# BGU-CS-VIL/DPMMSubClusters.jl

Hardware: AMD Instinct MI355X
Metric: Gibbs iterations/sec, N=10M D=64 NIW (higher is better)
Workload: dtype f32

## Files before the change

### dpmmsubclusters.jl_amd/binding.py

```python
import ctypes
import os
import subprocess

import numpy as np

_HERE = os.path.dirname(os.path.abspath(__file__))
PRIOR_NIW, PRIOR_MULT = 0, 1
MAX_CLUSTERS = 1024

_c_i64p = ctypes.POINTER(ctypes.c_int64)
_c_f32p = ctypes.POINTER(ctypes.c_float)
_c_f64p = ctypes.POINTER(ctypes.c_double)

ABI = [
    ("dpmm_abi_version", ctypes.c_int, []),
    ("dpmm_create", ctypes.c_int, [ctypes.POINTER(ctypes.c_void_p), ctypes.c_int, ctypes.c_int, ctypes.c_int64, ctypes.c_int64, ctypes.c_int, ctypes.c_uint64]),
    ("dpmm_destroy", ctypes.c_int, [ctypes.c_void_p]),
    ("dpmm_last_error", ctypes.c_char_p, [ctypes.c_void_p]),
    ("dpmm_upload_points", ctypes.c_int, [ctypes.c_void_p, _c_f32p, ctypes.c_int64]),
    ("dpmm_upload_points_device", ctypes.c_int, [ctypes.c_void_p, ctypes.c_void_p, ctypes.c_int64]),
    ("dpmm_upload_points_npy", ctypes.c_int, [ctypes.c_void_p, ctypes.c_void_p, ctypes.c_int, ctypes.c_int64, ctypes.c_int]),
    ("dpmm_upload_points_csc", ctypes.c_int, [ctypes.c_void_p, _c_i64p, _c_i64p, _c_f32p, ctypes.c_int]),
    ("dpmm_init_labels", ctypes.c_int, [ctypes.c_void_p, ctypes.c_int, ctypes.c_uint32]),
    ("dpmm_set_labels", ctypes.c_int, [ctypes.c_void_p, _c_i64p, _c_i64p]),
# ... 72 lines not shown
    ("dpmm_comm_allgather_host", ctypes.c_int, [ctypes.c_void_p, ctypes.c_void_p, ctypes.c_int64, ctypes.c_void_p]),
]

ABI_TENSOR = [
    ("dpmm_upload_points_strided_device", ctypes.c_int, [ctypes.c_void_p, ctypes.c_void_p, ctypes.c_int, ctypes.c_int64, ctypes.c_int64, ctypes.c_int]),
    ("dpmm_get_points_device", ctypes.c_int, [ctypes.c_void_p, ctypes.c_void_p, ctypes.c_int64]),
    ("dpmm_get_labels_device", ctypes.c_int, [ctypes.c_void_p, ctypes.c_void_p, ctypes.c_void_p]),
    ("dpmm_set_labels_device", ctypes.c_int, [ctypes.c_void_p, ctypes.c_void_p, ctypes.c_void_p]),
    ("dpmm_predict_points_device", ctypes.c_int, [ctypes.c_void_p, ctypes.c_void_p, ctypes.c_void_p]),
]
DT_F16, DT_BF16, DT_F32, DT_F64, DT_U8, DT_I16, DT_I32, DT_I64 = range(8)

HOST_ALLREDUCE_FN = ctypes.CFUNCTYPE(ctypes.c_int, ctypes.c_void_p, ctypes.c_void_p, ctypes.c_int64, ctypes.c_int)

MASTER_NSCALARS = 8
OPT_SCREEN_MARGIN, OPT_TAIL_SCREEN, OPT_PRESCREEN, OPT_ORDERED_SWEEP, OPT_MULT_FORCE_F32, OPT_STATS_ITEMS, OPT_STATS_GROUPS, OPT_TRACE_SLOW, OPT_LOGLIK_REF_CONST, OPT_WAVE_PRIO, OPT_MULT_NO_U8, OPT_SWEEP_GRID, OPT_SWEEP_QUEUE_ROUNDS, OPT_BALL_SCREEN, OPT_KERNEL_TIMING, OPT_STATS_DERIVE, OPT_NOISE_AHEAD, OPT_REF_BRACKET, OPT_SORT_TILE, OPT_ONE_COLLECTIVE, OPT_BF16_SCREENS, OPT_COMM_TIMEOUT_MS, OPT_DIRECTION_SCREEN, _OPT_RESERVED_24, OPT_MULT_DRAWS_AHEAD, OPT_B3_SUBLABELS, OPT_LEAN_TILES, OPT_MASTER_POLL, OPT_CHAIN_FUSION, OPT_LEAN_DIRECTION, OPT_PAIR_BALL = range(1, 32)


class DpmmError(RuntimeError):
    def __init__(self, code, msg):
        super().__init__(f"libdpmmhip error {code}: {msg}")
        self.code = code


def lib_path():
    return os.path.join(_HERE, "lib", "libdpmmhip.so")


def locked_make(args, lock_dir):
    import fcntl
    os.makedirs(lock_dir, exist_ok=True)
# ... 541 lines not shown
```

### dpmmsubclusters.jl_amd/csrc/dpmm_api.cpp

```cpp
#include "../../include/dpmm_hip.h"
#include "../../include/dpmm_hip_master.h"
#include "../../include/dpmm_hip_debug.h"
#include "../../include/dpmm_hip_tensor.h"

#include <hip/hip_runtime.h>
#include <dlfcn.h>

#include <algorithm>
#include <atomic>
#include <condition_variable>
#include <mutex>
#include <thread>
#include <chrono>
#include <cmath>
#include <cstdio>
#include <cstring>
#include <cstdlib>
#include <ctime>
#include <string>
#include <unordered_map>
#include <vector>

#include "dpmm_kernels.h"

// ... 114 lines not shown
    int sel_all_ones = 0, sel_capacity = 0;
    long long *d_counts64 = nullptr;
    float *d_malpha = nullptr;
    bool mult_master = false, mult_has_alpha1 = false;
    int rows_full_K = -1;
    double mult_prior_c[4] = {0, 0, 0, 0};
    int32_t *d_mpairs = nullptr;
    std::vector<int32_t> mpairs_req, mpairs_shadow;
    bool marg_req = false, marg_valid = false;
    int marg_req_outlier = 0, marg_K = 0, marg_np = 0;
    double *h_marg = nullptr;
    double *d_ccache = nullptr;
    bool cache_force = true;
    int cache_K = -1;
    int opt_derive = 1;
    int64_t dbg_early_wait = 0;
    int opt_noise_ahead = -1;
    bool master = false;
    NiwMasterArgs ma{};
    double *d_m0 = nullptr, *d_psi_lo = nullptr, *d_pairs = nullptr;
    double *d_Y[2] = {nullptr, nullptr};
    float *d_mu_draw[2] = {nullptr, nullptr};
    int draw_cur = 0;
    size_t pair_cap = 0;
    float *d_ld_sigma[2] = {nullptr, nullptr};
    int master_slots = 0, master_K = 0;
    hipStream_t stream2 = nullptr;
    hipEvent_t ev_master = nullptr, ev_spec = nullptr;
    hipEvent_t ev_noise = nullptr;
    hipEvent_t ev_pairs = nullptr;
// ... 145 lines not shown
    return e;
}

static int ensure_pinned(dpmm_ctx *c, size_t bytes) {
    if (bytes <= c->h_pin_bytes) return DPMM_OK;
    HIPCHK(c, sync_stream(c, c->stream));
    if (c->h_pin) hipHostFree(c->h_pin);
    c->h_pin = nullptr; c->h_pin_bytes = 0;
    size_t cap = 1 << 20;
    while (cap < bytes) cap *= 2;
    HIPCHK(c, hipHostMalloc((void **)&c->h_pin, cap, hipHostMallocDefault));
    c->h_pin_bytes = cap;
    return DPMM_OK;
}

static int fail(dpmm_ctx *c, int code, const std::string &msg) {
    if (c) c->err = msg; else g_create_error = msg;
    return code;
}

struct UidByValue { char internal[128]; };
namespace {
struct Rccl {
    void *handle = nullptr;
    int (*GetUniqueId)(void *) = nullptr;
    int (*CommInitRank)(void **, int,  UidByValue, int) = nullptr;
    int (*CommDestroy)(void *) = nullptr;
    int (*CommAbort)(void *) = nullptr;
    int (*AllReduce)(const void *, void *, size_t, int, int, void *, hipStream_t) = nullptr;
    int (*AllGather)(const void *, void *, size_t, int, void *, hipStream_t) = nullptr;
// ... 507 lines not shown
        if (int rc2 = pack_sparse_image(c, c->d_raw, c->d_Rp, c->K)) return rc2;
        c->rp_current = false;
        c->mspec_valid = false;
        HIPCHK(c, sync_stream(c, c->stream));
    }
    c->have_points = true;
    c->cache_force = true;
    c->rows_full_K = -1;
    return DPMM_OK;
}

int dpmm_init_labels(dpmm_ctx *c, int init_clusters, uint32_t epoch) {
    if (!c) return DPMM_EINVAL;
    if (init_clusters < 1 || init_clusters > DPMM_MAX_CLUSTERS) return fail(c, DPMM_ELIMIT, "init_clusters out of range");
    HIPCHK(c, hipSetDevice(c->device));
    if (c->n > 0) HIPCHK(c, launch_init_labels(c->dbins, c->n, c->first, init_clusters, 0, c->seed, epoch, c->stream));
    c->have_labels = true;
    c->rows_full_K = -1;
    return DPMM_OK;
}

int dpmm_init_labels_from(dpmm_ctx *c, int init_clusters, int first_label, uint32_t epoch) {
    if (!c) return DPMM_EINVAL;
    if (first_label < 1 || init_clusters < 1 || first_label - 1 + init_clusters > DPMM_MAX_CLUSTERS) return fail(c, DPMM_ELIMIT, "init_clusters / first_label out of range");
    HIPCHK(c, hipSetDevice(c->device));
    if (c->n > 0) HIPCHK(c, launch_init_labels(c->dbins, c->n, c->first, init_clusters, first_label - 1, c->seed, epoch, c->stream));
    c->have_labels = true;
    c->rows_full_K = -1;
    return DPMM_OK;
}

int dpmm_set_labels(dpmm_ctx *c, const int64_t *labels, const int64_t *sub) {
    if (!c) return DPMM_EINVAL;
    if (!c->have_labels && (!labels || !sub)) return fail(c, DPMM_ESTATE, "first dpmm_set_labels must provide both vectors");
    HIPCHK(c, hipSetDevice(c->device));
    if (c->n == 0) { c->have_labels = true; return DPMM_OK; }
    int64_t *tmp = nullptr;
    HIPCHK(c, hipMalloc(&tmp, sizeof(int64_t) * 2 * (size_t)c->n));
    int rc = DPMM_OK;
    hipError_t e = hipSuccess;
    if (labels) e = hipMemcpyAsync(tmp, labels, sizeof(int64_t) * c->n, hipMemcpyHostToDevice, c->stream);
    if (e == hipSuccess && sub) e = hipMemcpyAsync(tmp + c->n, sub, sizeof(int64_t) * c->n, hipMemcpyHostToDevice, c->stream);
    if (e == hipSuccess) e = launch_bins_from_i64(c->dbins, labels ? tmp : nullptr, sub ? tmp + c->n : nullptr, c->n, c->stream);
    if (e == hipSuccess) e = sync_stream(c, c->stream);
    hipFree(tmp);
    if (e != hipSuccess) { c->err = std::string("dpmm_set_labels: ") + hipGetErrorString(e); rc = DPMM_EHIP; }
    else c->have_labels = true;
    c->rows_full_K = -1;
    return rc;
}

int dpmm_get_labels(dpmm_ctx *c, int64_t *labels, int64_t *sub) {
    if (!c) return DPMM_EINVAL;
    if (!c->have_labels) return fail(c, DPMM_ESTATE, "labels not initialised");
    HIPCHK(c, hipSetDevice(c->device));
    if (c->n == 0) return DPMM_OK;
    int64_t *tmp = nullptr;
// ... 279 lines not shown
    for (char *p = bus; *p; ++p) if (*p >= 'A' && *p <= 'F') *p = (char)(*p - 'A' + 'a');
    const std::string path = std::string("/sys/bus/pci/devices/") + bus + "/numa_node";
    FILE *f = fopen(path.c_str(), "r");
    if (!f) return -1;
    int node = -1;
    if (fscanf(f, "%d", &node) != 1) node = -1;
    fclose(f);
    return node;
}

static int noise_flush(dpmm_ctx *c);
static int run_sweep(dpmm_ctx *c, uint32_t epoch, int final_argmax, float *table, int64_t table_stride) {
    if (!c->have_points || !c->have_params) return fail(c, DPMM_ESTATE, "sweep needs points and parameters");
    HIPCHK(c, hipSetDevice(c->device));
    if (c->n == 0) return DPMM_OK;
    if (c->prior == DPMM_PRIOR_NIW && !table) {
        if (!c->work_zeroed) HIPCHK(c, hipMemsetAsync(c->d_work, 0, sizeof(unsigned long long) * DPMM_WORK_SLOTS, c->stream));
        c->work_zeroed = false;
    }
    if (!table && (c->opt_timing & 1)) HIPCHK(c, hipEventRecord(c->ev[0], c->stream));
    if (c->prior == DPMM_PRIOR_NIW) {
        NiwSweepArgs a{};
        a.X = c->dX; a.ldx = c->ldx; a.n = c->n; a.first_index = c->first; a.ntiles = c->ntiles; a.K = c->K;
        a.Rp = c->d_Rp; a.mup = c->d_mup; a.cst = c->d_cst;
        a.tdf = c->predictive ? c->d_tdf : nullptr;
        a.scratch = table ? table : c->d_scratch;
        a.scratch_stride = table ? table_stride : c->scratch_stride;
        a.scratch_by_tile = table ? 1 : 0;
        a.labels_only = table ? 1 : 0;
        a.bins = c->dbins; a.seed = c->seed; a.epoch = epoch; a.final_argmax = final_argmax;
// ... 47 lines not shown
            if (parts && !c->ev_part[0]) for (auto &e : c->ev_part) HIPCHK(c, hipEventCreate(&e));
            if (use_lean) {
                const size_t hw = hard_list_words(c->n);
                uint32_t *mine = c->d_hard + (size_t)c->hard_flip * hw, *other = c->d_hard + (size_t)(c->hard_flip ^ 1) * hw;
                c->hard_flip ^= 1;
                c->lean_ran = true;
                uint32_t *need2 = a.need ? c->h_need + 8 * (size_t)c->sweep_grid_max : nullptr;
                const bool al = a.order != nullptr && c->perm_nbins > 0 && c->perm_nbins <= NIW_LEAN_MAX_BINS;
                uint32_t *need3 = a.need ? c->h_need + 12 * (size_t)c->sweep_grid_max : nullptr;
                NiwSweepArgs al_args = a;
                if (!c->opt_lean_dir) { al_args.sp_frag = nullptr; al_args.sp_cons = nullptr; }
                if (c->have_pb && c->opt_pair_ball && al_args.ball) al_args.ball |= 2;
                HIPCHK(c, launch_niw_lean(al_args, mine, need2, other, al ? c->sb.bin_start : nullptr, al ? c->perm_nbins : 0, need3, c->sweep_grid, c->stream));
                if (parts) HIPCHK(c, hipEventRecord(c->ev_part[0], c->stream));
                list = mine;
            }
            a.bf16scr |= 4;
            a.tdf = reinterpret_cast<const float *>(list);
            const float *mdist_kept = a.mdist;
            if (list) a.mdist = reinterpret_cast<const float *>(c->h_hard);
            HIPCHK(c, launch_niw_sweep(c->NB, a, c->sweep_grid, c->stream));
            a.mdist = mdist_kept;
            if (parts) HIPCHK(c, hipEventRecord(c->ev_part[1], c->stream));
            c->have_parts = parts ? (use_lean ? 2 : 1) : 0;
            a.bf16scr &= 3;
            a.tdf = nullptr;
            if (!list) HIPCHK(c, launch_niw_sub(a, nullptr, nullptr, c->sweep_grid, c->stream));
        } else {
            HIPCHK(c, launch_niw_sweep(c->NB, a, c->sweep_grid, c->stream));
            if (!table) c->have_parts = 0;
// ... 140 lines not shown
    HIPCHK(c, sync_stream(c, c->stream));
    c->rows_late = false;
    if (c->h_out) hipHostFree(c->h_out);
    c->h_out = nullptr; c->h_out_bytes = 0;
    size_t cap = 1 << 20;
    while (cap < bytes) cap *= 2;
    HIPCHK(c, hipHostMalloc((void **)&c->h_out, cap, hipHostMallocDefault));
    c->h_out_bytes = cap;
    return DPMM_OK;
}

static int flush_undo(dpmm_ctx *c) {
    if (!c->undo_pending) return DPMM_OK;
    c->undo_pending = false;
    const uint8_t *flags = reinterpret_cast<const uint8_t *>(c->d_out) + sizeof(double) * 2 * (size_t)c->K * (size_t)c->packed_stride;
    HIPCHK(c, launch_niw_undo_reset(c->dbins, c->n, c->K, flags, c->d_cside, c->stream));
    return DPMM_OK;
}
static int run_stats(dpmm_ctx *c, const int64_t *idx, int n_idx, bool with_reset = false, uint32_t reset_epoch = 0, uint8_t *flags_to = nullptr,
                     bool *flags_sent = nullptr) {
    if (!c->have_points || !c->have_labels || c->K < 1) return fail(c, DPMM_ESTATE, "suffstats need points, labels and parameters (K)");
    HIPCHK(c, hipSetDevice(c->device));
    const int nbins = 2 * c->K;
    c->marg_valid = false;
    c->mspec_valid = false;
    const bool one_auto = c->packed_stride <= 4096;
    const bool one_coll = with_reset && comm_attached(c) && (c->opt_one_collective < 0 ? one_auto : c->opt_one_collective != 0);
    c->last_pass_one_collective = one_coll;
    if (c->opt_timing & 2) HIPCHK(c, hipEventRecord(c->ev[2], c->stream));
    if (idx) {
// ... 10 lines not shown
        c->sel_all_ones = 0;
    } else if (with_reset && c->n > 0 && c->opt_derive) {
    } else if (c->sel_all_ones < nbins) {
        HIPCHK(c, hipMemsetAsync(c->sb.bin_sel, 1, c->sel_capacity, c->stream));
        c->sel_all_ones = c->sel_capacity;
    }
    bool derive = false;
    StatsArgs a{};
    a.X = c->dX; a.ldx = c->ldx; a.n = c->n; a.D = c->D; a.nbins = nbins; a.chunk = c->chunk;
    a.max_items = (int)((c->n + c->chunk - 1) / c->chunk) + nbins;
    a.range_groups = c->opt_stats_groups;
    a.sb = c->sb; a.slabs = c->d_slabs; a.slab_stride = c->slab_stride; a.out = (one_coll && c->prior == DPMM_PRIOR_NIW) ? c->d_red : c->d_out; a.packed_stride = c->packed_stride; a.row_off = c->d_row_off; a.inv_off = c->d_inv_off;
    if (with_reset && c->n > 0) {
        const bool fold_reset = (c->opt_chain & 8) != 0 && (c->n >= 4000000 || (c->opt_chain & 32) != 0) && nbins <= STEP_SPEC_MAX_BINS &&
                                c->sb.tile_spec != nullptr && c->sb.spec_bins != nullptr;
        HIPCHK(c, launch_step_hist(c->dbins, c->n, nbins, c->sb, c->stream, fold_reset ? 1 : 0, c->first, c->seed, reset_epoch));
        const long long *gc = nullptr;
        if (comm_attached(c) && !one_coll) {
            HIPCHK(c, launch_widen_counts(c->sb.fast_total, FAST_TOTAL_STRIDE, c->d_counts64, nbins, c->stream));
            if (int rc = comm_allreduce(c, c->d_counts64, nbins, 0)) return rc;
            gc = c->d_counts64;
        }
        uint8_t *flags = reinterpret_cast<uint8_t *>(c->d_out) + sizeof(double) * (size_t)nbins * (size_t)c->packed_stride;
        if (!fold_reset) HIPCHK(c, launch_step_reset(c->dbins, c->n, c->first, nbins, c->sb, gc, flags, c->K, c->seed, reset_epoch, one_coll ? c->d_cside : nullptr, c->stream));
        derive = c->opt_derive != 0;
        const int force_all = (c->cache_force || c->cache_K != c->K) ? 1 : 0;
        const StepReset rs{gc, flags, c->K, one_coll ? c->d_cside : nullptr, c->first, c->seed, reset_epoch};
        HIPCHK(c, launch_step_scan_scatter(c->dbins, a, derive ? 1 : 0, force_all, c->opt_chain & 1, fold_reset ? &rs : nullptr, c->stream));
        if (derive) { c->sel_all_ones = 0; c->cache_force = false; c->cache_K = c->K; }
    } else {
        if (c->n > 0) {
// ... 313 lines not shown
static bool master_marks_left(const double *sm, int K) { return master_records_marked(sm, 3 * (int64_t)K); }
static void master_mark_records(double *sm, int64_t nrec) {
    for (int64_t r = 0; r < nrec; ++r)
        for (int e = 0; e < 5; ++e) std::memcpy(&sm[r * DPMM_MASTER_NSCALARS + e], &MASTER_MARK, 8);
}
static int wait_master_records(dpmm_ctx *c, const double *sm, int64_t nrec, const double *pr, int64_t npr) {
    const bool armed = c->watchdog && c->coll_pending;
    if (armed) wd_arm(c);
    int rc = DPMM_OK;
    const auto t0 = std::chrono::steady_clock::now();
    auto next_query = t0 + std::chrono::milliseconds(1);
    std::chrono::steady_clock::time_point drained{};
    bool is_drained = false;
    for (uint64_t spin = 0;; ++spin) {
        if (!master_records_marked(sm, nrec) && !(npr > 0 && master_records_marked(pr, npr))) break;
        __builtin_ia32_pause();
        if ((spin & 63u) != 63u) continue;
        if (c->comm_aborted.load(std::memory_order_relaxed)) break;
        const auto now = std::chrono::steady_clock::now();
        if (now < next_query) continue;
        next_query = now + std::chrono::milliseconds(1);
        const hipError_t q = hipStreamQuery(c->stream);
        if (q == hipSuccess) {
            if (!is_drained) { is_drained = true; drained = now; ++c->dbg_early_wait; }
            else if (now - drained > std::chrono::seconds(5)) { rc = fail(c, DPMM_EHIP, "posterior records missing 5 s after the stream drained"); break; }
        } else if (q != hipErrorNotReady) { c->err = std::string("hipStreamQuery while waiting for the posteriors: ") + hipGetErrorString(q); rc = DPMM_EHIP; break; }
    }
    if (armed && wd_disarm(c)) {
        c->err = "collective timed out: a peer rank is gone or stuck (communicator aborted after DPMM_OPT_COMM_TIMEOUT_MS)";
        return DPMM_ECOMM;
    }
// ... 578 lines not shown
    }
    if (int rc = ensure_pinned(c, sizeof(int32_t) * h.size())) return rc;
    HIPCHK(c, sync_stream(c, c->stream));
    memcpy(c->h_pin, h.data(), sizeof(int32_t) * h.size());
    HIPCHK(c, launch_copy_bytes(c->d_small, c->h_pin, sizeof(int32_t) * h.size(), c->stream));
    return DPMM_OK;
}

int dpmm_split(dpmm_ctx *c, const int64_t *idx, const int64_t *new_idx, int n, uint32_t epoch) {
    if (!c) return DPMM_EINVAL;
    if (!c->have_labels) return fail(c, DPMM_ESTATE, "labels not initialised");
    if (n == 0) return DPMM_OK;
    if (!idx || !new_idx) return fail(c, DPMM_EINVAL, "null index list");
    HIPCHK(c, hipSetDevice(c->device));
    if (int rc = upload_idx(c, idx, new_idx, n, DPMM_MAX_CLUSTERS)) return rc;
    if (c->n > 0) HIPCHK(c, launch_split(c->dbins, c->n, c->first, c->d_small, n, c->seed, epoch, c->stream));
    c->rows_full_K = -1;
    return DPMM_OK;
}

int dpmm_merge(dpmm_ctx *c, const int64_t *idx, const int64_t *new_idx, int n) {
    if (!c) return DPMM_EINVAL;
    if (!c->have_labels) return fail(c, DPMM_ESTATE, "labels not initialised");
    if (n == 0) return DPMM_OK;
    if (!idx || !new_idx) return fail(c, DPMM_EINVAL, "null index list");
    HIPCHK(c, hipSetDevice(c->device));
    if (int rc = upload_idx(c, idx, new_idx, n, DPMM_MAX_CLUSTERS)) return rc;
    if (c->n > 0) HIPCHK(c, launch_merge(c->dbins, c->n, c->d_small, n, c->stream));
    c->rows_full_K = -1;
    return DPMM_OK;
}

int dpmm_remove_empty(dpmm_ctx *c, const int64_t *pts_count, int K) {
    if (!c) return DPMM_EINVAL;
    if (!c->have_labels) return fail(c, DPMM_ESTATE, "labels not initialised");
    if (!pts_count || K < 1 || K > DPMM_MAX_CLUSTERS) return fail(c, DPMM_EINVAL, "bad pts_count / K");
    HIPCHK(c, hipSetDevice(c->device));
    std::vector<int32_t> map(DPMM_MAX_CLUSTERS);
    for (int l = 1; l <= DPMM_MAX_CLUSTERS; ++l) {
        int v = l, removed = 0;
        for (int k = 1; k <= K; ++k)
            if (pts_count[k - 1] == 0) {
                if (v > k - removed) v -= 1;
                removed += 1;
            }
        map[l - 1] = v - 1;
    }
    if (int rc = ensure_pinned(c, sizeof(int32_t) * map.size())) return rc;
    HIPCHK(c, sync_stream(c, c->stream));
    memcpy(c->h_pin, map.data(), sizeof(int32_t) * map.size());
    HIPCHK(c, launch_copy_bytes(c->d_small, c->h_pin, sizeof(int32_t) * map.size(), c->stream));
    if (c->n > 0) HIPCHK(c, launch_remap(c->dbins, c->n, c->d_small, c->stream));
    c->rows_full_K = -1;
    return DPMM_OK;
}

int dpmm_reset_sublabels(dpmm_ctx *c, const int64_t *idx, int n, uint32_t epoch) {
    if (!c) return DPMM_EINVAL;
    if (!c->have_labels) return fail(c, DPMM_ESTATE, "labels not initialised");
    HIPCHK(c, hipSetDevice(c->device));
    if (idx) {
        if (n == 0) return DPMM_OK;
        if (int rc = upload_idx(c, idx, nullptr, n, DPMM_MAX_CLUSTERS)) return rc;
    }
    if (c->n > 0) HIPCHK(c, launch_reset_sub(c->dbins, c->n, c->first, idx ? c->d_small : nullptr, idx ? n : 0, c->seed, epoch, c->stream));
    c->rows_full_K = -1;
    return DPMM_OK;
}

static int smart_buffers(dpmm_ctx *c) {
    if (c->d_proj) return DPMM_OK;
    const size_t n = (size_t)std::max<int64_t>(c->n, 1);
    HIPCHK(c, hipMalloc(&c->d_proj, sizeof(double) * n));
    HIPCHK(c, hipMalloc(&c->d_vals, sizeof(double) * n));
    HIPCHK(c, hipMalloc(&c->d_smart, sizeof(double) * (4 * (size_t)smart_groups() + 8 + 2 * (size_t)c->D)));
    return DPMM_OK;
}
static int smart_check(dpmm_ctx *c, int64_t cluster) {
    if (!c->have_points || !c->have_labels) return fail(c, DPMM_ESTATE, "smart split needs points and labels");
// ... 29 lines not shown
    HIPCHK(c, hipSetDevice(c->device));
    out4[0] = out4[1] = out4[2] = out4[3] = 0.;
    if (c->n == 0) return DPMM_OK;
    double *d_out = c->d_smart + 4 * (size_t)smart_groups();
    HIPCHK(c, launch_smart_kmeans(c->dbins, c->d_proj, c->n, (int)(cluster - 1), m_lo, m_hi, c->d_smart, d_out, c->stream));
    HIPCHK(c, hipMemcpyAsync(out4, d_out, sizeof(double) * 4, hipMemcpyDeviceToHost, c->stream));
    HIPCHK(c, sync_stream(c, c->stream));
    return DPMM_OK;
}

int dpmm_smart_assign(dpmm_ctx *c, int64_t cluster, double m_lo, double m_hi) {
    if (!c) return DPMM_EINVAL;
    if (int rc = smart_check(c, cluster)) return rc;
    if (!c->d_proj) return fail(c, DPMM_ESTATE, "dpmm_smart_project has not been called");
    HIPCHK(c, hipSetDevice(c->device));
    if (c->n > 0) HIPCHK(c, launch_smart_assign(c->dbins, c->d_proj, c->n, (int)(cluster - 1), m_lo, m_hi, c->stream));
    return DPMM_OK;
}

int dpmm_set_ground_truth(dpmm_ctx *c, const int64_t *gt, int n_gt) {
    if (!c) return DPMM_EINVAL;
    if ((!gt && c->n > 0) || n_gt < 1 || n_gt > 65536) return fail(c, DPMM_EINVAL, "bad ground truth");
    HIPCHK(c, hipSetDevice(c->device));
    if (!c->d_gt) HIPCHK(c, hipMalloc(&c->d_gt, sizeof(int32_t) * (size_t)std::max<int64_t>(c->n, 1)));
    if (c->d_cont) { hipFree(c->d_cont); c->d_cont = nullptr; }
    HIPCHK(c, hipMalloc(&c->d_cont, sizeof(unsigned long long) * (size_t)DPMM_MAX_CLUSTERS * n_gt));
    if (c->n > 0) {
        int64_t *tmp = nullptr;
        HIPCHK(c, hipMalloc(&tmp, sizeof(int64_t) * (size_t)c->n));
        hipError_t e = hipMemcpyAsync(tmp, gt, sizeof(int64_t) * c->n, hipMemcpyHostToDevice, c->stream);
// ... 49 lines not shown
            if (c->have_points) return fail(c, DPMM_ESTATE, "DPMM_OPT_MULT_FORCE_F32 must be set before the points are uploaded");
            c->opt_force_f32 = value != 0; return DPMM_OK;
        case DPMM_OPT_STATS_ITEMS:
            if (c->Kcap > 0) return fail(c, DPMM_ESTATE, "DPMM_OPT_STATS_ITEMS must be set before the first parameters / K");
            if (value >= 1) c->chunk_dense = c->chunk = (int)std::max<int64_t>((c->prior == DPMM_PRIOR_NIW && c->D <= 64) ? 32 : 256, ((c->n + (int64_t)value - 1) / (int64_t)value + 3) / 4 * 4);
            if (c->x_sparse) return set_points_chunk(c, true);
            return DPMM_OK;
        case DPMM_OPT_STATS_GROUPS: c->opt_stats_groups = value > 0 ? (int)value : 0; return DPMM_OK;
        case DPMM_OPT_TRACE_SLOW: c->opt_trace = value != 0; return DPMM_OK;
        case DPMM_OPT_LOGLIK_REF_CONST: c->opt_ref_const = value != 0; return DPMM_OK;
        case DPMM_OPT_WAVE_PRIO: c->opt_prio = value != 0; return DPMM_OK;
        case DPMM_OPT_MULT_DRAWS_AHEAD: c->opt_mult_draws_ahead = value != 0; c->mspec_valid = false; return DPMM_OK;
        case DPMM_OPT_SWEEP_QUEUE_ROUNDS: c->opt_queue_rounds = value < 0 ? -1 : (int)value; return DPMM_OK;
        case DPMM_OPT_BALL_SCREEN: c->opt_ball = value != 0; return DPMM_OK;
        case DPMM_OPT_STATS_DERIVE: c->opt_derive = value != 0; c->cache_force = true; return DPMM_OK;
        case DPMM_OPT_NOISE_AHEAD: c->opt_noise_ahead = value < 0 ? -1 : (value != 0); return DPMM_OK;
        case DPMM_OPT_REF_BRACKET: c->opt_bracket = value != 0; return DPMM_OK;
        case DPMM_OPT_COMM_TIMEOUT_MS: c->comm_timeout_ms = value > 0 ? (int)std::min(value, 2.0e9) : 0; return DPMM_OK;
        case DPMM_OPT_BF16_SCREENS: c->opt_bf16scr = value != 0; return DPMM_OK;
        case DPMM_OPT_MASTER_POLL: c->opt_master_poll = value != 0; return DPMM_OK;
        case DPMM_OPT_PAIR_BALL: c->opt_pair_ball = value != 0; if (!c->opt_pair_ball) c->have_pb = false; return DPMM_OK;
        case DPMM_OPT_LEAN_DIRECTION: c->opt_lean_dir = value != 0; c->lean_off = 0; c->lean_backoff = 15; c->lean_ran = false; return DPMM_OK;
        case DPMM_OPT_CHAIN_FUSION: c->opt_chain = value < 0 ? (0x7fffffff & ~(8 | 32)) : (int)value; return DPMM_OK;
        case DPMM_OPT_LEAN_TILES: c->opt_lean = value != 0; c->lean_off = 0; c->lean_backoff = 15; c->lean_ran = false; return DPMM_OK;
        case DPMM_OPT_B3_SUBLABELS: c->opt_b3 = value != 0; if (!c->opt_b3) c->have_b3 = false; return DPMM_OK;
        case DPMM_OPT_DIRECTION_SCREEN:
            c->opt_direction = value < 0 ? -1 : (value != 0);
            if (c->opt_direction == 0) { c->sp_ready = false; c->sp_regime = false; }
            return DPMM_OK;
        case DPMM_OPT_ONE_COLLECTIVE: c->opt_one_collective = value < 0 ? -1 : (value != 0); return DPMM_OK;
// ... 430 lines not shown
    HIPCHK(c, launch_bins_to_i64(c->dbins, d_labels, d_sub, c->n, c->stream));
    HIPCHK(c, sync_stream(c, c->stream));
    return DPMM_OK;
}

int dpmm_set_labels_device(dpmm_ctx *c, const int64_t *d_labels, const int64_t *d_sub) {
    static const char *fn = "dpmm_set_labels_device";
    if (!c) return tensor_no_ctx(fn);
    if (!c->have_labels && (!d_labels || !d_sub)) return fail(c, DPMM_ESTATE, "first dpmm_set_labels_device must provide both vectors");
    HIPCHK(c, hipSetDevice(c->device));
    if (c->n == 0) { c->have_labels = true; return DPMM_OK; }
    const uint64_t bytes = sizeof(int64_t) * (uint64_t)c->n;
    if (d_labels) if (int rc = check_device_extent(c, fn, "d_labels", d_labels, bytes, sizeof(int64_t))) return rc;
    if (d_sub) if (int rc = check_device_extent(c, fn, "d_sub", d_sub, bytes, sizeof(int64_t))) return rc;
    if (d_labels || d_sub) {
        HIPCHK(c, launch_bins_from_i64(c->dbins, d_labels, d_sub, c->n, c->stream));
        HIPCHK(c, sync_stream(c, c->stream));
    }
    c->have_labels = true;
    c->rows_full_K = -1;
    return DPMM_OK;
}

int dpmm_predict_points_device(dpmm_ctx *c, int64_t *d_labels, float *d_probs) {
    static const char *fn = "dpmm_predict_points_device";
    if (!c) return tensor_no_ctx(fn);
    if (!c->predictive) return fail(c, DPMM_ESTATE, "dpmm_predict_points_device needs dpmm_set_predictive_* first");
    if (!c->have_points || !c->have_params) return fail(c, DPMM_ESTATE, "predict needs points and parameters");
    HIPCHK(c, hipSetDevice(c->device));
    if (c->n == 0) return DPMM_OK;
// ... 20 lines not shown
```

### dpmmsubclusters.jl_amd/csrc/dpmm_kernels.h

```cpp
#pragma once
#include <hip/hip_runtime.h>
#include <stdint.h>

#define DPMM_MAX_CLUSTERS_K 1024

namespace dpmm {


constexpr int DPMM_WORK_QUEUES = 8;
constexpr int DPMM_WORK_SLOTS = 8 + 16 * DPMM_WORK_QUEUES;
constexpr int DPMM_WORK_PER_WAVE = 8;
constexpr int REFB_FRAGS = 6, REFB_WORDS = REFB_FRAGS * 256;
constexpr int B3_WORDS = 3 * REFB_WORDS;
constexpr int B3_DVEC = 64;

struct NiwSweepArgs {
    const float *X;
    int64_t ldx;
    int64_t n;
    int64_t first_index;
    int64_t ntiles;
    int K;
    const float *Rp;
    const float *mup;
// ... 153 lines not shown
    unsigned *ticket;
    uint16_t *prev_lab;
    uint8_t *cdirty;
    uint8_t *cmode;
    int32_t *bin_total;
    int32_t *bin_start;
    int32_t *perm;
    int32_t *item_start;
    uint8_t *bin_sel;
    int32_t *perm_total;
};

hipError_t launch_sort_by_bin(const int32_t *bins, int64_t n, int nbins, const SortBufs &b, hipStream_t s);
constexpr int STEP_SPEC_MAX_BINS = 512;
struct StepReset { const long long *global_counts; uint8_t *flags; int K; uint8_t *cside; int64_t first; uint64_t seed; uint32_t epoch; };
hipError_t launch_step_hist(const int32_t *bins, int64_t n, int nbins, const SortBufs &b, hipStream_t s, int spec = 0, int64_t first = 0, uint64_t seed = 0, uint32_t epoch = 0);
hipError_t launch_step_reset(int32_t *bins, int64_t n, int64_t first, int nbins, const SortBufs &b, const long long *global_counts, uint8_t *flags,
                             int K, uint64_t seed, uint32_t epoch, uint8_t *cside, hipStream_t s);
hipError_t launch_onecoll_rows(const double *rows, double *red, int64_t stride, int K, const uint8_t *cside, uint8_t *flags, hipStream_t s);
hipError_t launch_niw_finalize_rows(const double *red, double *out, int64_t stride, int K, const uint8_t *cside, uint8_t *flags, uint8_t *flags_host, hipStream_t s);
hipError_t launch_niw_undo_reset(int32_t *bins, int64_t n, int K, const uint8_t *flags, const uint8_t *cside, hipStream_t s);
struct StatsArgs;
hipError_t launch_sort_finish(const int32_t *bins, const StatsArgs &a, hipStream_t s);
hipError_t launch_step_scan_scatter(int32_t *bins, const StatsArgs &a, int derive, int force_all, int fused_starts, const StepReset *rs, hipStream_t s);
hipError_t launch_derive_rows(double *out, double *cache, const uint8_t *mode, uint8_t *dirty, int64_t stride, int K, const uint8_t *flags_src,
                              uint8_t *flags_dst, hipStream_t s);

struct StatsArgs {
    const float *X;
    int64_t ldx;
    int64_t n;
// ... 71 lines not shown
```

### dpmmsubclusters.jl_amd/csrc/suffstats.hip

```cpp
#include <algorithm>
#include <cstdlib>
#include "dpmm_device.h"
#include "dpmm_kernels.h"

namespace dpmm {

typedef double f64x4 __attribute__((ext_vector_type(4)));
typedef float f32x4 __attribute__((ext_vector_type(4)));

template <int TILE, int W, bool SPEC>
__global__ __launch_bounds__(64 * W) void hist_kernel(const int32_t *__restrict__ bins, int64_t n, int nbins, int nt,
                                                      int32_t *__restrict__ tile_hist, int32_t *__restrict__ fast_total,
                                                      uint16_t *__restrict__ prev_lab, uint8_t *__restrict__ dirty,
                                                      int32_t *__restrict__ tile_spec, int32_t *__restrict__ spec_bins, int64_t first, uint64_t seed, uint32_t epoch) {
    extern __shared__ int cnt_all[];
    const int lane = threadIdx.x & 63, wave = threadIdx.x >> 6;
    int *const cnt = cnt_all + wave * nbins;
    const int tile = blockIdx.x * W + wave;
    for (int b = lane; b < nbins; b += 64) cnt[b] = 0;
    __syncthreads();
    const int64_t base = (int64_t)tile * TILE;
    int4 v[TILE / 256];
#pragma unroll
    for (int it = 0; it < TILE / 256; ++it) v[it] = make_int4(-1, -1, -1, -1);
    if (tile < nt) {
    auto track = [&](int64_t i, int bv) {
        const bool inr = (unsigned)bv < (unsigned)nbins;
        const unsigned z = inr ? (unsigned)bv >> 1 : 0xFFFFu, p = prev_lab[i];
        if (z != p) {
            if (inr) dirty[z] = 1;
// ... 472 lines not shown
        else if (m == 1) l[e] = c[e] - r[e];
        else r[e] = c[e] - l[e];
    }
    if (blockIdx.x == 0 && threadIdx.x == 0) { dirty[k] = 0; if (k == 0) dirty[DPMM_MAX_CLUSTERS_K] = 0; }
}
hipError_t launch_derive_rows(double *out, double *cache, const uint8_t *mode, uint8_t *dirty, int64_t stride, int K, const uint8_t *flags_src,
                              uint8_t *flags_dst, hipStream_t s) {
    DPMM_LAUNCH(derive_rows_kernel, dim3((unsigned)((stride + 255) / 256), K), dim3(256), 0, s, out, cache, mode, dirty, stride, K, flags_src, flags_dst);
    return hipGetLastError();
}

#define DPMM_TILE_DISPATCH(tile, CALL512, CALL2048) do { if ((tile) == 512) { CALL512; } else { CALL2048; } } while (0)
static inline int sort_nt(int64_t n, const SortBufs &b) { return (int)((n + b.tile - 1) / b.tile); }
template <int TILE>
static inline void launch_hist(const int32_t *bins, int64_t n, int nbins, int nt, int32_t *tile_cnt, int32_t *fast_total, uint16_t *prev_lab, uint8_t *dirty,
                               hipStream_t s, int32_t *tile_spec = nullptr, int32_t *spec_bins = nullptr, int64_t first = 0, uint64_t seed = 0, uint32_t epoch = 0) {
    if (tile_spec && nbins <= STEP_SPEC_MAX_BINS)
        DPMM_LAUNCH((hist_kernel<TILE, 8, true>), dim3((nt + 7) / 8), dim3(512), 16 * nbins * sizeof(int), s, bins, n, nbins, nt, tile_cnt, fast_total, prev_lab, dirty,
                    tile_spec, spec_bins, first, seed, epoch);
    else if (nbins <= 1024) DPMM_LAUNCH((hist_kernel<TILE, 8, false>), dim3((nt + 7) / 8), dim3(512), 8 * nbins * sizeof(int), s, bins, n, nbins, nt, tile_cnt, fast_total, prev_lab, dirty,
                                        (int32_t *)nullptr, (int32_t *)nullptr, (int64_t)0, (uint64_t)0, 0u);
    else DPMM_LAUNCH((hist_kernel<TILE, 1, false>), dim3(nt), dim3(64), nbins * sizeof(int), s, bins, n, nbins, nt, tile_cnt, fast_total, prev_lab, dirty,
                     (int32_t *)nullptr, (int32_t *)nullptr, (int64_t)0, (uint64_t)0, 0u);
}
hipError_t launch_sort_by_bin(const int32_t *bins, int64_t n, int nbins, const SortBufs &b, hipStream_t s) {
    const int nt = sort_nt(n, b);
    if (nt == 0) return hipSuccess;
    DPMM_TILE_DISPATCH(b.tile,
        launch_hist<512>(bins, n, nbins, nt, b.tile_cnt, (int32_t *)nullptr, (uint16_t *)nullptr, (uint8_t *)nullptr, s),
        launch_hist<2048>(bins, n, nbins, nt, b.tile_cnt, (int32_t *)nullptr, (uint16_t *)nullptr, (uint8_t *)nullptr, s));
    DPMM_LAUNCH(scan_tiles_kernel, dim3(nbins), dim3(256), 0, s, b.tile_cnt, b.tile_hist, nt, b.bin_total);
    return hipGetLastError();
}
hipError_t launch_step_hist(const int32_t *bins, int64_t n, int nbins, const SortBufs &b, hipStream_t s, int spec, int64_t first, uint64_t seed, uint32_t epoch) {
    const int nt = sort_nt(n, b);
    uint8_t *dirty = b.prev_lab ? b.cdirty : (uint8_t *)nullptr;
    int32_t *ts = (spec && b.tile_spec && b.spec_bins && nbins <= STEP_SPEC_MAX_BINS) ? b.tile_spec : (int32_t *)nullptr;
    DPMM_TILE_DISPATCH(b.tile,
        launch_hist<512>(bins, n, nbins, nt, b.tile_cnt, b.fast_total, b.prev_lab, dirty, s, ts, b.spec_bins, first, seed, epoch),
        launch_hist<2048>(bins, n, nbins, nt, b.tile_cnt, b.fast_total, b.prev_lab, dirty, s, ts, b.spec_bins, first, seed, epoch));
    return hipGetLastError();
}
hipError_t launch_step_reset(int32_t *bins, int64_t n, int64_t first, int nbins, const SortBufs &b, const long long *global_counts, uint8_t *flags,
                             int K, uint64_t seed, uint32_t epoch, uint8_t *cside, hipStream_t s) {
    const int nt = sort_nt(n, b);
    const size_t lds = nbins * sizeof(int) + ((K + 3) & ~3);
    DPMM_TILE_DISPATCH(b.tile,
        DPMM_LAUNCH(reset_recount_kernel<512>, dim3(nt), dim3(64), lds, s, bins, n, first, nbins, nt, b.fast_total, global_counts, b.tile_cnt, flags, K, seed, epoch, cside),
        DPMM_LAUNCH(reset_recount_kernel<2048>, dim3(nt), dim3(256), lds, s, bins, n, first, nbins, nt, b.fast_total, global_counts, b.tile_cnt, flags, K, seed, epoch, cside));
    return hipGetLastError();
}

#ifndef DPMM_STATS16_SB
#define DPMM_STATS16_SB 4
#endif
// ... 646 lines not shown
```

### include/dpmm_hip.h

```cpp
#ifndef DPMM_HIP_H
#define DPMM_HIP_H

#include <stddef.h>
#include <stdint.h>

#ifdef __cplusplus
extern "C" {
#endif

#define DPMM_ABI_VERSION 3

typedef struct dpmm_ctx dpmm_ctx;

enum { DPMM_PRIOR_NIW = 0, DPMM_PRIOR_MULT = 1 };

enum {
    DPMM_OK = 0,
    DPMM_EINVAL = -1,
    DPMM_ENODEVICE = -2,
    DPMM_EHIP = -3,
    DPMM_ESTATE = -4,
    DPMM_ELIMIT = -5,
    DPMM_ECOMM = -6
};
// ... 11 lines not shown
    DPMM_OPT_MULT_NO_U8 = 11,
    DPMM_OPT_SWEEP_GRID = 12,
    DPMM_OPT_SWEEP_QUEUE_ROUNDS = 13,
    DPMM_OPT_BALL_SCREEN = 14,
    DPMM_OPT_STATS_DERIVE = 16,
    DPMM_OPT_NOISE_AHEAD = 17,
    DPMM_OPT_REF_BRACKET = 18,
    DPMM_OPT_SORT_TILE = 19,
    DPMM_OPT_COMM_TIMEOUT_MS = 22,
    DPMM_OPT_B3_SUBLABELS = 26,
    DPMM_OPT_LEAN_TILES = 27,
    DPMM_OPT_MASTER_POLL = 28,
    DPMM_OPT_CHAIN_FUSION = 29,
    DPMM_OPT_LEAN_DIRECTION = 30,
    DPMM_OPT_PAIR_BALL = 31,
    DPMM_OPT_MULT_DRAWS_AHEAD = 25,
    DPMM_OPT_DIRECTION_SCREEN = 23,
    DPMM_OPT_BF16_SCREENS = 21,
    DPMM_OPT_ONE_COLLECTIVE = 20,
    DPMM_OPT_KERNEL_TIMING = 15,
    DPMM_OPT_WAVE_PRIO = 10
};

#define DPMM_MAX_CLUSTERS 1024
#define DPMM_MAX_DIM_NIW 256
#define DPMM_MAX_DIM_MULT_SPARSE 65536

int dpmm_abi_version(void);

int dpmm_create(dpmm_ctx **ctx, int prior_kind, int D, int64_t n_local, int64_t first_index,
// ... 77 lines not shown
```

Before: 700.0.

## Skip prev-label tracking in histogram when sweep reports no label changes

Adds a 'still labels' mechanism. The sweep's lean change list is recorded, and when its count is zero the step histogram kernel skips reading and writing the prev_lab and dirty tracking arrays. Every label-writing entry point now disarms this state so the stale-list assumption cannot be used after external label edits. The aim is to cut memory traffic in the hist pass on iterations where no labels moved. The cost is extra state coupling between sweep and step_stats, and a correctness risk if some label-writing path is missed.

```diff
diff --git a/dpmmsubclusters.jl_amd/binding.py b/dpmmsubclusters.jl_amd/binding.py
--- a/dpmmsubclusters.jl_amd/binding.py
+++ b/dpmmsubclusters.jl_amd/binding.py
@@ -110,7 +110,7 @@
 HOST_ALLREDUCE_FN = ctypes.CFUNCTYPE(ctypes.c_int, ctypes.c_void_p, ctypes.c_void_p, ctypes.c_int64, ctypes.c_int)
 
 MASTER_NSCALARS = 8
-OPT_SCREEN_MARGIN, OPT_TAIL_SCREEN, OPT_PRESCREEN, OPT_ORDERED_SWEEP, OPT_MULT_FORCE_F32, OPT_STATS_ITEMS, OPT_STATS_GROUPS, OPT_TRACE_SLOW, OPT_LOGLIK_REF_CONST, OPT_WAVE_PRIO, OPT_MULT_NO_U8, OPT_SWEEP_GRID, OPT_SWEEP_QUEUE_ROUNDS, OPT_BALL_SCREEN, OPT_KERNEL_TIMING, OPT_STATS_DERIVE, OPT_NOISE_AHEAD, OPT_REF_BRACKET, OPT_SORT_TILE, OPT_ONE_COLLECTIVE, OPT_BF16_SCREENS, OPT_COMM_TIMEOUT_MS, OPT_DIRECTION_SCREEN, _OPT_RESERVED_24, OPT_MULT_DRAWS_AHEAD, OPT_B3_SUBLABELS, OPT_LEAN_TILES, OPT_MASTER_POLL, OPT_CHAIN_FUSION, OPT_LEAN_DIRECTION, OPT_PAIR_BALL = range(1, 32)
+OPT_SCREEN_MARGIN, OPT_TAIL_SCREEN, OPT_PRESCREEN, OPT_ORDERED_SWEEP, OPT_MULT_FORCE_F32, OPT_STATS_ITEMS, OPT_STATS_GROUPS, OPT_TRACE_SLOW, OPT_LOGLIK_REF_CONST, OPT_WAVE_PRIO, OPT_MULT_NO_U8, OPT_SWEEP_GRID, OPT_SWEEP_QUEUE_ROUNDS, OPT_BALL_SCREEN, OPT_KERNEL_TIMING, OPT_STATS_DERIVE, OPT_NOISE_AHEAD, OPT_REF_BRACKET, OPT_SORT_TILE, OPT_ONE_COLLECTIVE, OPT_BF16_SCREENS, OPT_COMM_TIMEOUT_MS, OPT_DIRECTION_SCREEN, _OPT_RESERVED_24, OPT_MULT_DRAWS_AHEAD, OPT_B3_SUBLABELS, OPT_LEAN_TILES, OPT_MASTER_POLL, OPT_CHAIN_FUSION, OPT_LEAN_DIRECTION, OPT_PAIR_BALL, OPT_STILL_LABELS = range(1, 33)
 
 
 class DpmmError(RuntimeError):
diff --git a/dpmmsubclusters.jl_amd/csrc/dpmm_api.cpp b/dpmmsubclusters.jl_amd/csrc/dpmm_api.cpp
--- a/dpmmsubclusters.jl_amd/csrc/dpmm_api.cpp
+++ b/dpmmsubclusters.jl_amd/csrc/dpmm_api.cpp
@@ -152,6 +152,10 @@
     bool cache_force = true;
     int cache_K = -1;
     int opt_derive = 1;
+    int opt_still = 1;
+    bool still_armed = false;
+    int still_K = 0;
+    const uint32_t *still_list = nullptr;
     int64_t dbg_early_wait = 0;
     int opt_noise_ahead = -1;
     bool master = false;
@@ -327,6 +331,7 @@
     return DPMM_OK;
 }
 
+static inline void labels_written(dpmm_ctx *c) { c->still_armed = false; c->still_list = nullptr; }
 static int fail(dpmm_ctx *c, int code, const std::string &msg) {
     if (c) c->err = msg; else g_create_error = msg;
     return code;
@@ -864,6 +869,7 @@
     if (!c) return DPMM_EINVAL;
     if (init_clusters < 1 || init_clusters > DPMM_MAX_CLUSTERS) return fail(c, DPMM_ELIMIT, "init_clusters out of range");
     HIPCHK(c, hipSetDevice(c->device));
+    labels_written(c);
     if (c->n > 0) HIPCHK(c, launch_init_labels(c->dbins, c->n, c->first, init_clusters, 0, c->seed, epoch, c->stream));
     c->have_labels = true;
     c->rows_full_K = -1;
@@ -874,6 +880,7 @@
     if (!c) return DPMM_EINVAL;
     if (first_label < 1 || init_clusters < 1 || first_label - 1 + init_clusters > DPMM_MAX_CLUSTERS) return fail(c, DPMM_ELIMIT, "init_clusters / first_label out of range");
     HIPCHK(c, hipSetDevice(c->device));
+    labels_written(c);
     if (c->n > 0) HIPCHK(c, launch_init_labels(c->dbins, c->n, c->first, init_clusters, first_label - 1, c->seed, epoch, c->stream));
     c->have_labels = true;
     c->rows_full_K = -1;
@@ -891,6 +898,7 @@
     hipError_t e = hipSuccess;
     if (labels) e = hipMemcpyAsync(tmp, labels, sizeof(int64_t) * c->n, hipMemcpyHostToDevice, c->stream);
     if (e == hipSuccess && sub) e = hipMemcpyAsync(tmp + c->n, sub, sizeof(int64_t) * c->n, hipMemcpyHostToDevice, c->stream);
+    labels_written(c);
     if (e == hipSuccess) e = launch_bins_from_i64(c->dbins, labels ? tmp : nullptr, sub ? tmp + c->n : nullptr, c->n, c->stream);
     if (e == hipSuccess) e = sync_stream(c, c->stream);
     hipFree(tmp);
@@ -1200,6 +1208,8 @@
     if (!c->have_points || !c->have_params) return fail(c, DPMM_ESTATE, "sweep needs points and parameters");
     HIPCHK(c, hipSetDevice(c->device));
     if (c->n == 0) return DPMM_OK;
+    const bool still_was_armed = c->still_armed && c->still_K == c->K;
+    labels_written(c);
     if (c->prior == DPMM_PRIOR_NIW && !table) {
         if (!c->work_zeroed) HIPCHK(c, hipMemsetAsync(c->d_work, 0, sizeof(unsigned long long) * DPMM_WORK_SLOTS, c->stream));
         c->work_zeroed = false;
@@ -1277,6 +1287,7 @@
                 HIPCHK(c, launch_niw_lean(al_args, mine, need2, other, al ? c->sb.bin_start : nullptr, al ? c->perm_nbins : 0, need3, c->sweep_grid, c->stream));
                 if (parts) HIPCHK(c, hipEventRecord(c->ev_part[0], c->stream));
                 list = mine;
+                if (still_was_armed && c->opt_still) c->still_list = mine;
             }
             a.bf16scr |= 4;
             a.tdf = reinterpret_cast<const float *>(list);
@@ -1447,6 +1458,7 @@
     if (!c->undo_pending) return DPMM_OK;
     c->undo_pending = false;
     const uint8_t *flags = reinterpret_cast<const uint8_t *>(c->d_out) + sizeof(double) * 2 * (size_t)c->K * (size_t)c->packed_stride;
+    labels_written(c);
     HIPCHK(c, launch_niw_undo_reset(c->dbins, c->n, c->K, flags, c->d_cside, c->stream));
     return DPMM_OK;
 }
@@ -1487,7 +1499,10 @@
     if (with_reset && c->n > 0) {
         const bool fold_reset = (c->opt_chain & 8) != 0 && (c->n >= 4000000 || (c->opt_chain & 32) != 0) && nbins <= STEP_SPEC_MAX_BINS &&
                                 c->sb.tile_spec != nullptr && c->sb.spec_bins != nullptr;
-        HIPCHK(c, launch_step_hist(c->dbins, c->n, nbins, c->sb, c->stream, fold_reset ? 1 : 0, c->first, c->seed, reset_epoch));
+        const uint32_t *still = (c->opt_still && c->still_K == c->K) ? c->still_list : nullptr;
+        HIPCHK(c, launch_step_hist(c->dbins, c->n, nbins, c->sb, c->stream, fold_reset ? 1 : 0, c->first, c->seed, reset_epoch, still));
+        labels_written(c);
+        c->still_armed = c->sb.prev_lab != nullptr; c->still_K = c->K;
         const long long *gc = nullptr;
         if (comm_attached(c) && !one_coll) {
             HIPCHK(c, launch_widen_counts(c->sb.fast_total, FAST_TOTAL_STRIDE, c->d_counts64, nbins, c->stream));
@@ -1831,7 +1846,9 @@
     bool is_drained = false;
     for (uint64_t spin = 0;; ++spin) {
         if (!master_records_marked(sm, nrec) && !(npr > 0 && master_records_marked(pr, npr))) break;
+#if defined(__x86_64__) || defined(__i386__)
         __builtin_ia32_pause();
+#endif
         if ((spin & 63u) != 63u) continue;
         if (c->comm_aborted.load(std::memory_order_relaxed)) break;
         const auto now = std::chrono::steady_clock::now();
@@ -2440,6 +2457,7 @@
     if (!idx || !new_idx) return fail(c, DPMM_EINVAL, "null index list");
     HIPCHK(c, hipSetDevice(c->device));
     if (int rc = upload_idx(c, idx, new_idx, n, DPMM_MAX_CLUSTERS)) return rc;
+    labels_written(c);
     if (c->n > 0) HIPCHK(c, launch_split(c->dbins, c->n, c->first, c->d_small, n, c->seed, epoch, c->stream));
     c->rows_full_K = -1;
     return DPMM_OK;
@@ -2452,6 +2470,7 @@
     if (!idx || !new_idx) return fail(c, DPMM_EINVAL, "null index list");
     HIPCHK(c, hipSetDevice(c->device));
     if (int rc = upload_idx(c, idx, new_idx, n, DPMM_MAX_CLUSTERS)) return rc;
+    labels_written(c);
     if (c->n > 0) HIPCHK(c, launch_merge(c->dbins, c->n, c->d_small, n, c->stream));
     c->rows_full_K = -1;
     return DPMM_OK;
@@ -2476,6 +2495,7 @@
     HIPCHK(c, sync_stream(c, c->stream));
     memcpy(c->h_pin, map.data(), sizeof(int32_t) * map.size());
     HIPCHK(c, launch_copy_bytes(c->d_small, c->h_pin, sizeof(int32_t) * map.size(), c->stream));
+    labels_written(c);
     if (c->n > 0) HIPCHK(c, launch_remap(c->dbins, c->n, c->d_small, c->stream));
     c->rows_full_K = -1;
     return DPMM_OK;
@@ -2489,6 +2509,7 @@
         if (n == 0) return DPMM_OK;
         if (int rc = upload_idx(c, idx, nullptr, n, DPMM_MAX_CLUSTERS)) return rc;
     }
+    labels_written(c);
     if (c->n > 0) HIPCHK(c, launch_reset_sub(c->dbins, c->n, c->first, idx ? c->d_small : nullptr, idx ? n : 0, c->seed, epoch, c->stream));
     c->rows_full_K = -1;
     return DPMM_OK;
@@ -2548,6 +2569,7 @@
     if (int rc = smart_check(c, cluster)) return rc;
     if (!c->d_proj) return fail(c, DPMM_ESTATE, "dpmm_smart_project has not been called");
     HIPCHK(c, hipSetDevice(c->device));
+    labels_written(c);
     if (c->n > 0) HIPCHK(c, launch_smart_assign(c->dbins, c->d_proj, c->n, (int)(cluster - 1), m_lo, m_hi, c->stream));
     return DPMM_OK;
 }
@@ -2627,6 +2649,7 @@
         case DPMM_OPT_SWEEP_QUEUE_ROUNDS: c->opt_queue_rounds = value < 0 ? -1 : (int)value; return DPMM_OK;
         case DPMM_OPT_BALL_SCREEN: c->opt_ball = value != 0; return DPMM_OK;
         case DPMM_OPT_STATS_DERIVE: c->opt_derive = value != 0; c->cache_force = true; return DPMM_OK;
+        case DPMM_OPT_STILL_LABELS: c->opt_still = value != 0; labels_written(c); return DPMM_OK;
         case DPMM_OPT_NOISE_AHEAD: c->opt_noise_ahead = value < 0 ? -1 : (value != 0); return DPMM_OK;
         case DPMM_OPT_REF_BRACKET: c->opt_bracket = value != 0; return DPMM_OK;
         case DPMM_OPT_COMM_TIMEOUT_MS: c->comm_timeout_ms = value > 0 ? (int)std::min(value, 2.0e9) : 0; return DPMM_OK;
@@ -3087,6 +3110,7 @@
     if (d_labels) if (int rc = check_device_extent(c, fn, "d_labels", d_labels, bytes, sizeof(int64_t))) return rc;
     if (d_sub) if (int rc = check_device_extent(c, fn, "d_sub", d_sub, bytes, sizeof(int64_t))) return rc;
     if (d_labels || d_sub) {
+        labels_written(c);
         HIPCHK(c, launch_bins_from_i64(c->dbins, d_labels, d_sub, c->n, c->stream));
         HIPCHK(c, sync_stream(c, c->stream));
     }
diff --git a/dpmmsubclusters.jl_amd/csrc/dpmm_kernels.h b/dpmmsubclusters.jl_amd/csrc/dpmm_kernels.h
--- a/dpmmsubclusters.jl_amd/csrc/dpmm_kernels.h
+++ b/dpmmsubclusters.jl_amd/csrc/dpmm_kernels.h
@@ -191,7 +191,8 @@
 hipError_t launch_sort_by_bin(const int32_t *bins, int64_t n, int nbins, const SortBufs &b, hipStream_t s);
 constexpr int STEP_SPEC_MAX_BINS = 512;
 struct StepReset { const long long *global_counts; uint8_t *flags; int K; uint8_t *cside; int64_t first; uint64_t seed; uint32_t epoch; };
-hipError_t launch_step_hist(const int32_t *bins, int64_t n, int nbins, const SortBufs &b, hipStream_t s, int spec = 0, int64_t first = 0, uint64_t seed = 0, uint32_t epoch = 0);
+hipError_t launch_step_hist(const int32_t *bins, int64_t n, int nbins, const SortBufs &b, hipStream_t s, int spec = 0, int64_t first = 0, uint64_t seed = 0, uint32_t epoch = 0,
+                            const uint32_t *still = nullptr);
 hipError_t launch_step_reset(int32_t *bins, int64_t n, int64_t first, int nbins, const SortBufs &b, const long long *global_counts, uint8_t *flags,
                              int K, uint64_t seed, uint32_t epoch, uint8_t *cside, hipStream_t s);
 hipError_t launch_onecoll_rows(const double *rows, double *red, int64_t stride, int K, const uint8_t *cside, uint8_t *flags, hipStream_t s);
diff --git a/dpmmsubclusters.jl_amd/csrc/suffstats.hip b/dpmmsubclusters.jl_amd/csrc/suffstats.hip
--- a/dpmmsubclusters.jl_amd/csrc/suffstats.hip
+++ b/dpmmsubclusters.jl_amd/csrc/suffstats.hip
@@ -11,9 +11,11 @@
 template <int TILE, int W, bool SPEC>
 __global__ __launch_bounds__(64 * W) void hist_kernel(const int32_t *__restrict__ bins, int64_t n, int nbins, int nt,
                                                       int32_t *__restrict__ tile_hist, int32_t *__restrict__ fast_total,
-                                                      uint16_t *__restrict__ prev_lab, uint8_t *__restrict__ dirty,
-                                                      int32_t *__restrict__ tile_spec, int32_t *__restrict__ spec_bins, int64_t first, uint64_t seed, uint32_t epoch) {
+                                                      uint16_t *__restrict__ prev_lab_in, uint8_t *__restrict__ dirty,
+                                                      int32_t *__restrict__ tile_spec, int32_t *__restrict__ spec_bins, int64_t first, uint64_t seed, uint32_t epoch,
+                                                      const uint32_t *__restrict__ still) {
     extern __shared__ int cnt_all[];
+    uint16_t *const prev_lab = (still != nullptr && still[0] == 0u) ? (uint16_t *)nullptr : prev_lab_in;
     const int lane = threadIdx.x & 63, wave = threadIdx.x >> 6;
     int *const cnt = cnt_all + wave * nbins;
     const int tile = blockIdx.x * W + wave;
@@ -516,14 +518,15 @@
 static inline int sort_nt(int64_t n, const SortBufs &b) { return (int)((n + b.tile - 1) / b.tile); }
 template <int TILE>
 static inline void launch_hist(const int32_t *bins, int64_t n, int nbins, int nt, int32_t *tile_cnt, int32_t *fast_total, uint16_t *prev_lab, uint8_t *dirty,
-                               hipStream_t s, int32_t *tile_spec = nullptr, int32_t *spec_bins = nullptr, int64_t first = 0, uint64_t seed = 0, uint32_t epoch = 0) {
+                               hipStream_t s, int32_t *tile_spec = nullptr, int32_t *spec_bins = nullptr, int64_t first = 0, uint64_t seed = 0, uint32_t epoch = 0,
+                               const uint32_t *still = nullptr) {
     if (tile_spec && nbins <= STEP_SPEC_MAX_BINS)
         DPMM_LAUNCH((hist_kernel<TILE, 8, true>), dim3((nt + 7) / 8), dim3(512), 16 * nbins * sizeof(int), s, bins, n, nbins, nt, tile_cnt, fast_total, prev_lab, dirty,
-                    tile_spec, spec_bins, first, seed, epoch);
+                    tile_spec, spec_bins, first, seed, epoch, still);
     else if (nbins <= 1024) DPMM_LAUNCH((hist_kernel<TILE, 8, false>), dim3((nt + 7) / 8), dim3(512), 8 * nbins * sizeof(int), s, bins, n, nbins, nt, tile_cnt, fast_total, prev_lab, dirty,
-                                        (int32_t *)nullptr, (int32_t *)nullptr, (int64_t)0, (uint64_t)0, 0u);
+                                        (int32_t *)nullptr, (int32_t *)nullptr, (int64_t)0, (uint64_t)0, 0u, still);
     else DPMM_LAUNCH((hist_kernel<TILE, 1, false>), dim3(nt), dim3(64), nbins * sizeof(int), s, bins, n, nbins, nt, tile_cnt, fast_total, prev_lab, dirty,
-                     (int32_t *)nullptr, (int32_t *)nullptr, (int64_t)0, (uint64_t)0, 0u);
+                     (int32_t *)nullptr, (int32_t *)nullptr, (int64_t)0, (uint64_t)0, 0u, still);
 }
 hipError_t launch_sort_by_bin(const int32_t *bins, int64_t n, int nbins, const SortBufs &b, hipStream_t s) {
     const int nt = sort_nt(n, b);
@@ -534,13 +537,14 @@
     DPMM_LAUNCH(scan_tiles_kernel, dim3(nbins), dim3(256), 0, s, b.tile_cnt, b.tile_hist, nt, b.bin_total);
     return hipGetLastError();
 }
-hipError_t launch_step_hist(const int32_t *bins, int64_t n, int nbins, const SortBufs &b, hipStream_t s, int spec, int64_t first, uint64_t seed, uint32_t epoch) {
+hipError_t launch_step_hist(const int32_t *bins, int64_t n, int nbins, const SortBufs &b, hipStream_t s, int spec, int64_t first, uint64_t seed, uint32_t epoch,
+                            const uint32_t *still) {
     const int nt = sort_nt(n, b);
     uint8_t *dirty = b.prev_lab ? b.cdirty : (uint8_t *)nullptr;
     int32_t *ts = (spec && b.tile_spec && b.spec_bins && nbins <= STEP_SPEC_MAX_BINS) ? b.tile_spec : (int32_t *)nullptr;
     DPMM_TILE_DISPATCH(b.tile,
-        launch_hist<512>(bins, n, nbins, nt, b.tile_cnt, b.fast_total, b.prev_lab, dirty, s, ts, b.spec_bins, first, seed, epoch),
-        launch_hist<2048>(bins, n, nbins, nt, b.tile_cnt, b.fast_total, b.prev_lab, dirty, s, ts, b.spec_bins, first, seed, epoch));
+        launch_hist<512>(bins, n, nbins, nt, b.tile_cnt, b.fast_total, b.prev_lab, dirty, s, ts, b.spec_bins, first, seed, epoch, b.prev_lab ? still : nullptr),
+        launch_hist<2048>(bins, n, nbins, nt, b.tile_cnt, b.fast_total, b.prev_lab, dirty, s, ts, b.spec_bins, first, seed, epoch, b.prev_lab ? still : nullptr));
     return hipGetLastError();
 }
 hipError_t launch_step_reset(int32_t *bins, int64_t n, int64_t first, int nbins, const SortBufs &b, const long long *global_counts, uint8_t *flags,
diff --git a/include/dpmm_hip.h b/include/dpmm_hip.h
--- a/include/dpmm_hip.h
+++ b/include/dpmm_hip.h
@@ -49,6 +49,7 @@
     DPMM_OPT_CHAIN_FUSION = 29,
     DPMM_OPT_LEAN_DIRECTION = 30,
     DPMM_OPT_PAIR_BALL = 31,
+    DPMM_OPT_STILL_LABELS = 32,
     DPMM_OPT_MULT_DRAWS_AHEAD = 25,
     DPMM_OPT_DIRECTION_SCREEN = 23,
     DPMM_OPT_BF16_SCREENS = 21,
```

After: 705.3 (median of 6 runs). No clear change (+0.8%).
